# zjwzcx/A-2D-LiDAR-based-SLAM-System-for-Wheeled-Mobile-Robots

Measured on AMD Instinct MI355X. Metric: scans/sec (360-beam ICP + 0.05 m grid update), higher is better.
Workload: dtype f64; 1 GPU; configs[1]: 1000-scan replay (every 5th message of a 10 Hz stream, seed 1), 360 beams, ICP(max_iter=30, tol=0.001) + 400x400@0.05m grid, f64 point buffers; 32 independent replays of the 1000-scan trajectory per step (one slam_replay_dev call: ranges [32, 1000, 360], a map per trajectory); point_buffers=f64, pipeline=0, lanes=2, grid_mode=1, grid_group=16, parallelism=1 trajectory per GPU (32 independent replays of it per step)

## Files before the change

a-2d-lidar-based-slam-system-for-wheeled-mobile-robots_amd/csrc/grid_kernels.hip:

```cpp
#include <hip/hip_runtime.h>

#include <algorithm>
#include <mutex>
#include <utility>
#include <vector>
#include <climits>
#include <cstdio>
#include <cstdlib>
#include <type_traits>

#include "slam_internal.h"
#include "slam_stamps.h"
#include "grid_walk.h"

namespace slam {

__device__ __forceinline__ unsigned cast_ray(uint32_t *__restrict__ pass, uint32_t *__restrict__ hit, int xw, int yw,
                                             int pcx, int pcy, int pox, int poy, bool &first_pending)
{
    Ray r;
    first_pending = false;
    if (!ray_setup(pcx, pcy, pox, poy, r)) return 0u;
    unsigned nvis = 0;
    double error = 0.0;
// ... 448 lines not shown
    int x0 = any ? o[0] : 0, y0 = any ? o[1] : 0, W = any ? o[2] - o[0] + 1 : 0, H = any ? o[3] - o[1] + 1 : 0, cov = 1;
    if (any && !box_fits(o, win_cells)) {
        const int Hd = min(H, 192), Wd = min(W, win_cells / ((Hd + 1) & ~1));
        x0 = min(max(first.pcx - Wd / 2, o[0]), o[2] - Wd + 1);
        y0 = min(max(first.pcy - Hd / 2, o[1]), o[3] - Hd + 1) & ~ymask;
        W = Wd; H = Hd; cov = 0;
    }
    if ((long)W * ((H + 1) >> 1) > win_cells / 2) { atomicOr(g.status, kStatusGuard); W = 0; H = 0; cov = 0; }
    w[0] = x0; w[1] = y0; w[2] = W; w[3] = H; w[4] = cov;
}

__device__ __forceinline__ void flush_window(unsigned *win, uint32_t *pass, int yw, int wx0, int wy0, int W, int Hp2, bool pair64,
                                             bool zero = false)
{
    const int lane = threadIdx.x & 63, wave = threadIdx.x >> 6, nwaves = blockDim.x >> 6;
    const int rot = W > 0 ? (int)((blockIdx.x * 37u + blockIdx.y * 11u) % (unsigned)W) : 0;
    for (int rr = wave; rr < W; rr += nwaves) {
        const int row = rr + rot < W ? rr + rot : rr + rot - W;
        size_t gbase = (size_t)(wx0 + row) * yw + wy0;
        if (pair64 && (wy0 & 1) == 0) {
            for (int d = lane; d < Hp2; d += kWave) {
                unsigned v = win[row * Hp2 + d];
                if (zero) win[row * Hp2 + d] = 0u;
                if (v) atomicAdd(reinterpret_cast<unsigned long long *>(&pass[gbase + 2 * d]),
                                 (unsigned long long)(v & 0xffffu) | ((unsigned long long)(v >> 16) << 32));
            }
            continue;
        }
        for (int d = lane; d < Hp2; d += kWave) {
            unsigned v = win[row * Hp2 + d];
            if (zero) win[row * Hp2 + d] = 0u;
            unsigned p0 = v & 0xffffu, p1 = v >> 16;
            if (p0) atomicAdd(&pass[gbase + 2 * d], p0);
            if (p1) atomicAdd(&pass[gbase + 2 * d + 1], p1);
        }
    }
}

__device__ __forceinline__ void flush_hits(unsigned *win, unsigned short *park, int nrays, uint32_t *hit, int yw, int wx0, int wy0,
                                           int Hs)
{
    __syncthreads();
    for (int k = threadIdx.x; k < nrays; k += blockDim.x) {
        const unsigned c = park[k];
        if (c == kNoHit) continue;
        const unsigned sh = (c & 1u) * 16u;
        const unsigned old = atomicAdd(&win[c >> 1], 1u << sh);
        if ((old >> sh) & 0xffffu) park[k] = (unsigned short)kNoHit;
    }
    __syncthreads();
    for (int k = threadIdx.x; k < nrays; k += blockDim.x) {
        const unsigned c = park[k];
        if (c == kNoHit) continue;
        const unsigned tot = (win[c >> 1] >> ((c & 1u) * 16u)) & 0xffffu;
        const unsigned wx = c / (unsigned)Hs, wy = c - wx * (unsigned)Hs;
        atomicAdd(&hit[(size_t)(wx0 + (int)wx) * yw + (wy0 + (int)wy)], tot);
    }
}

__device__ __forceinline__ void sweep_strip(const unsigned *win, uint32_t *pass, int8_t *pm, int yw, int sx0, int wy0, int SW, int H,
                                            int qrow, unsigned qinv, uint32_t pthr)
{
    const int tid = threadIdx.x, lane = tid & 63, Hp2 = H >> 1, total = SW * qrow;
    constexpr int kBatch = 4;
    for (int q0 = tid; q0 < total; q0 += kBatch * blockDim.x) {
        uint4 p[kBatch];
        uint32_t om[kBatch], d0[kBatch], d1[kBatch];
        size_t at[kBatch];
        bool live[kBatch];
#pragma unroll
        for (int u = 0; u < kBatch; ++u) {
            const int q = q0 + u * (int)blockDim.x;
            d0[u] = d1[u] = 0u;
            if (q < total) {
                const int r = (int)__umulhi((unsigned)q, qinv), c = q - r * qrow;
                const uint2 d = *reinterpret_cast<const uint2 *>(win + (r * Hp2 + 2 * c));
                d0[u] = d.x; d1[u] = d.y;
                at[u] = (size_t)(sx0 + r) * yw + (wy0 + 4 * c);
            }
            const unsigned long long m = __ballot((d0[u] | d1[u]) != 0u);
            live[u] = ((m >> (lane & 60)) & 0xFull) != 0ull;
            if (live[u]) {
                p[u] = *reinterpret_cast<const uint4 *>(pass + at[u]);
                om[u] = *reinterpret_cast<const uint32_t *>(pm + at[u]);
            }
        }
#pragma unroll
        for (int u = 0; u < kBatch; ++u) {
            if (!live[u]) continue;
            const uint32_t d0v = d0[u], d1v = d1[u];
            p[u].x += d0v & 0x7fffu; p[u].y += (d0v >> 16) & 0x7fffu; p[u].z += d1v & 0x7fffu; p[u].w += (d1v >> 16) & 0x7fffu;
            *reinterpret_cast<uint4 *>(pass + at[u]) = p[u];
            if (!(d0v | d1v)) continue;
            const uint32_t o = om[u];
            const uint32_t tb = ((d0v & 0xffffu) ? 1u : 0u) | ((d0v >> 16) ? 0x100u : 0u) | ((d1v & 0xffffu) ? 0x10000u : 0u) | ((d1v >> 16) ? 0x1000000u : 0u);
            const uint32_t fb = ((d0v >> 15) & 1u) | (((d0v >> 31) & 1u) << 8) | (((d1v >> 15) & 1u) << 16) | ((d1v >> 31) << 24);
            const uint32_t was = (o >> 6) & 0x01010101u, fresh = (o >> 4) & 0x01010101u;
            const uint32_t pmax = max(max(p[u].x, p[u].y), max(p[u].z, p[u].w));
            if (((tb & ~was) & (fresh | fb)) != 0u || pmax >= pthr) {
                uint32_t occ = was | fb;
                occ |= (p[u].x >= pthr ? 1u : 0u) | (p[u].y >= pthr ? 0x100u : 0u) | (p[u].z >= pthr ? 0x10000u : 0u) | (p[u].w >= pthr ? 0x1000000u : 0u);
                const uint32_t tm = tb * 255u;
                const uint32_t out = (o & ~tm) | ((occ * 100u) & tm);
                if (out != o) *reinterpret_cast<uint32_t *>(pm + at[u]) = out;
            }
        }
    }
// ... 35 lines not shown
        ctl->phases = 1; ctl->parity = 0;
    }
    const bool sorted = nrays <= sort_cap;
    unsigned short *bins = reinterpret_cast<unsigned short *>(win);
    for (int k = tid; k < 4 * kSortBins; k += blockDim.x) hist[k] = 0;
    __syncthreads();
    STAMP(0);

    win_pass1(g, src, sc, l, s0, cnt, n, sorted, ctl->bbox, ctl->first_bad, [&](int r, int i, bool casts, int quad, int lbin) {
        bins[r] = casts ? (unsigned short)(lbin | (quad << 7) | ((i & 1) << 9)) : (unsigned short)0xffffu;
    });
    if (tid == 0) {
        const int *bb = ctl->bbox;
        if (bb[0] <= bb[2]) {
            int ox0 = INT_MAX, oy0 = INT_MAX, ox1 = INT_MIN, oy1 = INT_MIN;
            for (int k = 0; k < cnt; ++k) { ox0 = min(ox0, sc[k].pcx); ox1 = max(ox1, sc[k].pcx); oy0 = min(oy0, sc[k].pcy); oy1 = max(oy1, sc[k].pcy); }
            quadrant_boxes(bb, ox0, oy0, ox1, oy1, ctl->qbox);
        }
        auto fits = [&](unsigned mask) -> bool { int o[4]; return !box_of(ctl->qbox, mask, g.xw, g.yw, ymask, o) || box_fits(o, win_cells); };
        unsigned part[4] = {0u, 0u, 0u, 0u};
        int nph = 1, parity = 0;
        pick_parts(split != 0, my_half, sorted, fits, part, nph, parity);
        for (int q = 0; q < 4; ++q) ctl->phq[q] = -1;
        for (int ph = 0; ph < nph; ++ph) {
            for (int q = 0; q < 4; ++q)
                if (part[ph] >> q & 1u) ctl->phq[q] = ph;
            int o[4];
            const bool any = box_of(ctl->qbox, part[ph], g.xw, g.yw, ymask, o);
            fit_window(g, any, o, ymask, sc[0], win_cells, ctl->phw[ph]);
        }
        ctl->phases = nph; ctl->parity = parity;
        if (!sorted) { ctl->seg[0] = 0; ctl->seg[1] = nrays; }
    }
    __syncthreads();
    STAMP(1);
    const int phases = ctl->phases;
    if (sorted) {
        const bool parity = ctl->parity != 0;
        for (int r = tid; r < nrays; r += blockDim.x) {
            const unsigned b = bins[r];
            if (b == 0xffffu) continue;
            const int ph = ctl->phq[(b >> 7) & 3u];
            const bool mine = ph >= 0 && (!parity || (int)((b >> 9) & 1u) == my_half);
            const unsigned fin = (unsigned)ph * kSortBins + (b & 127u);
            bins[r] = mine ? (unsigned short)fin : (unsigned short)0xffffu;
            if (mine) atomicAdd(&hist[fin], 1);
        }
        __syncthreads();
        counting_sort<8>(hist, bins, lds.order, nrays, ctl->seg);
    }
    unsigned nvis = 0;
    int W = ctl->phw[0][2], H = ctl->phw[0][3];
    bool covers = ctl->phw[0][4] != 0;
    for (int ph = 0; ph < phases; ++ph) {
        const int seg0 = ctl->seg[ph], seg1 = ctl->seg[ph + 1];
        if (seg0 == seg1) continue;
        const int *o = ctl->phw[ph];
        const int wx0 = o[0], wy0 = o[1];
        W = o[2]; H = o[3]; covers = o[4] != 0;
        const int Hp2 = (H + 1) >> 1;
        __syncthreads();
        if (tid == 0) ctl->next_ray = 0;
        for (int w = tid; w < W * Hp2; w += blockDim.x) win[w] = 0u;
        __syncthreads();
        STAMP(2);
        const unsigned short *ord = sorted ? lds.order + seg0 : nullptr;
        unsigned short *park = sorted && lds_hits ? lds.order + seg0 : nullptr;
        if (covers) nvis += cast_rays<true>(g, src, sc, l, s0, n, seg1 - seg0, &ctl->next_ray, ord, win, wx0, wy0, W, H, Hp2, pass, hit, ctl->first_bad, park);
        else        nvis += cast_rays<false>(g, src, sc, l, s0, n, seg1 - seg0, &ctl->next_ray, ord, win, wx0, wy0, W, H, Hp2, pass, hit, ctl->first_bad, park);
        __syncthreads();
        STAMP(3);
        flush_window(win, pass, g.yw, wx0, wy0, W, Hp2, pair64, park != nullptr);
        if (park) flush_hits(win, park, seg1 - seg0, hit, g.yw, wx0, wy0, 2 * Hp2);
    }
    finish_workgroup(g, &ctl->visits, nvis, tid);
    STAMP(4);
    STAMP_VAL((ctl->parity << 8) | (covers ? 1 : 0) | (phases << 4) | ((unsigned)(W * ((H + 1) & ~1)) << 12));
    STAMP_END(5);
    lds_guard_check(lds.guard, g.status);
}

template <class Src>
__global__ void __launch_bounds__(1024) k_grid_update_own(GridDev g, Src src, int group_size, int sort_cap, int win_cells)
{
    extern __shared__ __attribute__((aligned(16))) char smem[];
    const WinLds lds(smem, group_size, sort_cap, win_cells);
    ScanConst *sc = lds.sc; WinCtl *ctl = lds.ctl; int *hist = lds.hist; unsigned *win = lds.win;
    lds_guard_fill(lds.guard);
    STAMP_DECL;

    const int tid = threadIdx.x, lane = tid & 63, wave = tid >> 6, nwaves = blockDim.x >> 6;
    const int l = blockIdx.y;
    const int s0 = (int)blockIdx.x * group_size;
    const int cnt = min(group_size, src.scans_per_traj() - s0);
    const int gi = src.own_grid(l);
    uint32_t *pass = g.pass + (size_t)gi * g.xw * g.yw, *hit = g.hit + (size_t)gi * g.xw * g.yw;
    int8_t *pm = g.pmap_live + (size_t)gi * g.xw * g.yw;
    const int n = src.n, nrays = cnt * n;

    const bool fused = (g.yw & 3) == 0 && (((size_t)gi * g.xw * g.yw) & 3) == 0;
    const bool pair64 = (g.yw & 1) == 0 && (((size_t)gi * g.xw * g.yw) & 1) == 0;
    const int ymask = fused ? 3 : pair64 ? 1 : 0;
    if (tid < cnt) { src.scan_const(l, s0 + tid, g, sc[tid]); ctl->first_bad[tid] = INT_MAX; }
    if (tid == 0) {
        ctl->bbox[0] = ctl->bbox[1] = INT_MAX; ctl->bbox[2] = ctl->bbox[3] = INT_MIN; ctl->next_ray = 0; ctl->visits = 0ull;
        ctl->strips = 0; ctl->strip_w = 0;
    }
    const bool sorted = nrays <= sort_cap;
    unsigned short *bins = reinterpret_cast<unsigned short *>(win);
    for (int k = tid; k < kSortBins; k += blockDim.x) hist[k] = 0;
    __syncthreads();
    STAMP(0);

    win_pass1(g, src, sc, l, s0, cnt, n, sorted, ctl->bbox, ctl->first_bad, [&](int r, int, bool, int, int lbin) {
        bins[r] = (unsigned short)lbin;
        atomicAdd(&hist[lbin], 1);
    });
    if (tid == 0) {
        int o[4] = {ctl->bbox[0], ctl->bbox[1], ctl->bbox[2], ctl->bbox[3]};
        int *w = ctl->phw[0];
        const bool any = clamp_box(g.xw, g.yw, o, 0);
        if (any && fused && cnt == 1 && nrays < 32768 && g.hit_levels == 1 && (g.yw & 15) == 0) {
            const int ya = o[1] & ~15, Ha = ((o[3] | 15) + 1) - ya, Wb = o[2] - o[0] + 1;
            int S = (int)(((long)Wb * Ha + win_cells - 1) / win_cells), Ws = (Wb + S - 1) / S;
            while ((long)Ws * Ha > win_cells && S < Wb) { ++S; Ws = (Wb + S - 1) / S; }
            if ((long)Ws * Ha <= win_cells) { w[0] = o[0]; w[1] = ya; w[2] = Wb; w[3] = Ha; w[4] = 1; ctl->strips = S; ctl->strip_w = Ws; }
// ... 1594 lines not shown
```

a-2d-lidar-based-slam-system-for-wheeled-mobile-robots_amd/csrc/icp_kernels.hip:

```cpp
#include <hip/hip_fp16.h>
#include <hip/hip_runtime.h>

#include <type_traits>

#include "slam_internal.h"
#include "slam_stamps.h"

namespace slam {

#ifdef SLAM_STAMPS_ICP
__device__ unsigned long long g_polar_lanes[6];
hipError_t debug_polar_lanes(unsigned long long out[6], bool clear)
{
    hipError_t e = hipMemcpyFromSymbol(out, HIP_SYMBOL(g_polar_lanes), sizeof(unsigned long long) * 6);
    if (e == hipSuccess && clear) {
        const unsigned long long zero[6] = {0ull, 0ull, 0ull, 0ull, 0ull, 0ull};
        e = hipMemcpyToSymbol(HIP_SYMBOL(g_polar_lanes), zero, sizeof zero);
    }
    return e;
}
#endif

__device__ __forceinline__ double ld(const double *p, long i) { return p[i]; }
__device__ __forceinline__ double ld(const float *p, long i) { return (double)p[i]; }
// ... 1485 lines not shown
    if (same[0] || same[1]) w[0] = w[1] = w[2] = w[3] = 0.0;
    if (tid == 0) {
        store_transform(T_out + 9 * (long)b, kabsch_from_sums(cax, cay, cbx, cby, w[0], w[1], w[2], w[3]));
    }
}

hipError_t launch_kabsch(const double *src, const double *tar, int B, int n, double *T_out, hipStream_t s)
{
    SLAM_LAUNCH(k_kabsch, dim3(B), dim3(256), 0, s, src, tar, n, T_out);
    return hipGetLastError();
}

template <typename T>
__global__ void __launch_bounds__(256) k_scan_to_points(const float *__restrict__ ranges, const double *__restrict__ cos_t,
                                                        const double *__restrict__ sin_t, long total, int n, int clip_inf,
                                                        T *__restrict__ pts)
{
    for (long e = (long)blockIdx.x * blockDim.x + threadIdx.x; e < total; e += (long)gridDim.x * blockDim.x) {
        long b = e / n;
        int i = (int)(e - b * n);
        double r = (double)ranges[e];
        if (clip_inf && r == INFINITY) r = 30.0;
        st(pts, b * 2 * n + i, cos_t[i] * r);
        st(pts, b * 2 * n + n + i, sin_t[i] * r);
    }
}

hipError_t launch_scan_to_points(const float *ranges, const double *cos_t, const double *sin_t, long total, int n,
                                 int clip_inf, int dtype, void *pts, hipStream_t s)
{
    long blocks = (total + 255) / 256;
    if (blocks > 4096) blocks = 4096;
    if (blocks < 1) blocks = 1;
    switch (dtype) {
    case SLAM_F64:
        SLAM_LAUNCH((k_scan_to_points<double>), dim3(blocks), dim3(256), 0, s, ranges, cos_t, sin_t, total, n, clip_inf, static_cast<double *>(pts));
        break;
    case SLAM_F32:
        SLAM_LAUNCH((k_scan_to_points<float>), dim3(blocks), dim3(256), 0, s, ranges, cos_t, sin_t, total, n, clip_inf, static_cast<float *>(pts));
        break;
    case SLAM_F16:
        SLAM_LAUNCH((k_scan_to_points<__half>), dim3(blocks), dim3(256), 0, s, ranges, cos_t, sin_t, total, n, clip_inf, static_cast<__half *>(pts));
        break;
    default: return hipErrorInvalidValue;
    }
    return hipGetLastError();
}

constexpr int kComposeChunk = 64;
constexpr int kComposeThreads = 256;
constexpr int kComposeBatch = 16;

__global__ void __launch_bounds__(kComposeThreads) k_pose_compose(const double *__restrict__ T, const double *__restrict__ pose0, int n,
                                                                  double *__restrict__ poses)
{
    __shared__ __attribute__((aligned(16))) double dyaw[3][kComposeChunk];
    __shared__ __attribute__((aligned(16))) double thb[2][kComposeChunk];
    __shared__ __attribute__((aligned(16))) double ab[2][kComposeChunk][4];
    __shared__ __attribute__((aligned(16))) double xo[2][2][kComposeChunk];
    __builtin_amdgcn_s_setprio(3);
    const int l = blockIdx.x, tid = threadIdx.x, lane = tid & 63, wave = tid >> 6;
    const double *Tl = T + 9 * (long)l * n;
    double *Pl = poses + 3 * (long)l * n;
    const int nc = (n + kComposeChunk - 1) / kComposeChunk;
    double th = pose0[3 * l + 2];
    double v = pose0[3 * l + (lane & 1)];
    auto load2 = [&](int chunk, int e0, int e1, double &u0, double &u1) {
        const int k = chunk * kComposeChunk + lane;
        const bool in = chunk >= 0 && chunk < nc && k < n;
        u0 = in ? Tl[9 * (long)k + e0] : 0.0;
        u1 = in ? Tl[9 * (long)k + e1] : 0.0;
    };
    double m0 = 0.0, m1 = 0.0;
    if (wave == 2) load2(0, 3, 0, m0, m1);
    if (wave == 3) load2(-2, 2, 5, m0, m1);
    for (int s = 0; s < nc + 4; ++s) {
        if (wave == 0) {
            const int c = s - 1;
            if (c >= 0 && c < nc && lane == 0) {
                const double2 *d2 = reinterpret_cast<const double2 *>(dyaw[c % 3]);
                double2 *o2 = reinterpret_cast<double2 *>(thb[c & 1]);
                double2 cur[kComposeBatch / 2], nxt[kComposeBatch / 2];
#pragma unroll
                for (int u = 0; u < kComposeBatch / 2; ++u) cur[u] = d2[u];
#pragma unroll
                for (int b0 = 0; b0 < kComposeChunk; b0 += kComposeBatch) {
                    if (b0 + kComposeBatch < kComposeChunk) {
#pragma unroll
                        for (int u = 0; u < kComposeBatch / 2; ++u) nxt[u] = d2[(b0 + kComposeBatch) / 2 + u];
                    }
#pragma unroll
                    for (int u = 0; u < kComposeBatch / 2; ++u) {
                        double2 o;
                        o.x = th; th = th + cur[u].x;
                        o.y = th; th = th + cur[u].y;
                        o2[b0 / 2 + u] = o;
                    }
#pragma unroll
                    for (int u = 0; u < kComposeBatch / 2; ++u) cur[u] = nxt[u];
                }
            }
        } else if (wave == 1) {
            const int c = s - 3;
            if (c >= 0 && c < nc && lane < 2) {
                const double2 *p2 = reinterpret_cast<const double2 *>(&ab[c & 1][0][0]) + lane;
                double2 *o2 = reinterpret_cast<double2 *>(xo[c & 1][lane]);
                double2 cur[kComposeBatch], nxt[kComposeBatch];
#pragma unroll
                for (int u = 0; u < kComposeBatch; ++u) cur[u] = p2[2 * u];
#pragma unroll
                for (int b0 = 0; b0 < kComposeChunk; b0 += kComposeBatch) {
                    if (b0 + kComposeBatch < kComposeChunk) {
#pragma unroll
                        for (int u = 0; u < kComposeBatch; ++u) nxt[u] = p2[2 * (b0 + kComposeBatch + u)];
                    }
#pragma unroll
                    for (int u = 0; u < kComposeBatch; u += 2) {
                        double2 o;
                        v = (v + cur[u].x) - cur[u].y;
                        o.x = v;
                        v = (v + cur[u + 1].x) - cur[u + 1].y;
                        o.y = v;
                        o2[(b0 + u) / 2] = o;
                    }
#pragma unroll
                    for (int u = 0; u < kComposeBatch; ++u) cur[u] = nxt[u];
                }
            }
        } else if (wave == 2) {
            double n0, n1;
            load2(s + 1, 3, 0, n0, n1);
            if (s < nc) dyaw[s % 3][lane] = (s * kComposeChunk + lane < n) ? atan2(m0, m1) : 0.0;
            m0 = n0; m1 = n1;
            const int c = s - 4, k = c * kComposeChunk + lane;
            if (c >= 0 && k < n) {
                Pl[3 * (long)k] = xo[c & 1][0][lane];
                Pl[3 * (long)k + 1] = xo[c & 1][1][lane];
            }
        } else {
            double n0, n1;
            load2(s - 1, 2, 5, n0, n1);
            const int c = s - 2, k = c * kComposeChunk + lane;
            if (c >= 0 && c < nc) {
                double a_ = 0.0, b_ = 0.0, c_ = 0.0, d_ = 0.0;
                if (k < n) {
                    const double h = thb[c & 1][lane];
                    const double cs = cos(h), sn = sin(h);
                    a_ = cs * m0; b_ = sn * m1; c_ = sn * m0; d_ = cs * m1;
                    Pl[3 * (long)k + 2] = h + dyaw[c % 3][lane];
                }
                double2 *q = reinterpret_cast<double2 *>(&ab[c & 1][lane][0]);
                q[0] = make_double2(a_, b_);
                q[1] = make_double2(c_, -d_);
            }
            m0 = n0; m1 = n1;
        }
        __syncthreads();
    }
}

__global__ void __launch_bounds__(256) k_pose_step(const double *__restrict__ T, const double *__restrict__ pose0,
                                                   const double *__restrict__ prior, int L, double *__restrict__ poses,
                                                   double *__restrict__ heading_cs)
{
    int l = blockIdx.x * blockDim.x + threadIdx.x;
    if (l >= L) return;
    const double *t = T + 9 * (long)l;
    double m00 = t[0], m10 = t[3], m02 = t[2], m12 = t[5];
    if (prior) {
        const double *p = prior + 6 * (long)l;
        m00 = t[0] * p[0] + t[1] * p[3];
        m10 = t[3] * p[0] + t[4] * p[3];
        m02 = t[0] * p[2] + t[1] * p[5] + t[2];
        m12 = t[3] * p[2] + t[4] * p[5] + t[5];
    }
    double x = pose0[3 * l], y = pose0[3 * l + 1], th = pose0[3 * l + 2];
    double dyaw = atan2(m10, m00);
    double c = cos(th), s = sin(th);
    poses[3 * l] = (x + c * m02) - s * m12;
    poses[3 * l + 1] = (y + s * m02) + c * m12;
    const double th1 = th + dyaw;
    poses[3 * l + 2] = th1;
    if (heading_cs) { heading_cs[2 * l] = cos(th1); heading_cs[2 * l + 1] = sin(th1); }
}

hipError_t launch_pose_compose(const double *T, const double *pose0, int L, int n, double *poses, hipStream_t s,
                               const double *prior, double *heading_cs)
{
    if (prior || heading_cs || (n == 1 && L > 64)) {
        if (n != 1) return hipErrorInvalidValue;
        SLAM_LAUNCH(k_pose_step, dim3((L + 255) / 256), dim3(256), 0, s, T, pose0, prior, L, poses, heading_cs);
        return hipGetLastError();
    }
    SLAM_LAUNCH(k_pose_compose, dim3(L), dim3(kComposeThreads), 0, s, T, pose0, n, poses);
    return hipGetLastError();
}

}
```

a-2d-lidar-based-slam-system-for-wheeled-mobile-robots_amd/csrc/slam_abi.hip:

```cpp
#include <hip/hip_runtime.h>

#include <algorithm>
#include <cmath>
#include <cstdarg>
#include <cstdio>
#include <cstring>
#include <string>
#include <initializer_list>
#include <mutex>
#include <utility>
#include <vector>

#include "slam_internal.h"
#include "slam_stamps.h"

using namespace slam;

namespace {

thread_local std::string g_err;

int fail(int code, const char *fmt, ...)
{
    char buf[512];
// ... 34 lines not shown
}

size_t align_up(size_t v, size_t a = 256) { return (v + a - 1) / a * a; }

struct Arena {
    char *base = nullptr;
    size_t cap = 0, used = 0;
};

struct Pending {
    int kind;
    hipEvent_t e0, e1;
    bool first;
};

}

struct slam_ctx {
    int device = 0;
    hipStream_t stream = nullptr;
    bool own_stream = false;
    Arena staging;
    Arena scratch;
    Arena tiles;
    char *pinned = nullptr;
    size_t pinned_cap = 0;
    int *status = nullptr;
    bool timing = false;
    unsigned timing_mask = ~0u;
    std::vector<hipEvent_t> pool;
    std::vector<Pending> pending;
    double ms[SLAM_K_COUNT] = {0};
    int64_t launches[SLAM_K_COUNT] = {0};
    int grid_mode = 1;
    int grid_group = 0;
    int grid_split = -1;
    int icp_qpt = 0;
    int replay_reset = 0;
    int icp_f32_filter = -1;
    int win_lds_hits = -1;
    int icp_one_wave = -1;
    int raycast_lds = -1;
    int mcl_shape = -1;
    int icp_team = 0;
    int pipeline = 0;
    hipStream_t gstream = nullptr;
    hipStream_t cstream = nullptr;
    hipEvent_t ev_fork = nullptr, ev_join = nullptr, ev_icp = nullptr, ev_pose = nullptr;
    hipEvent_t ev_cast[2] = {nullptr, nullptr};
    const void *cast_poses[2] = {nullptr, nullptr};
    const void *cast_T[2] = {nullptr, nullptr};
    double *pipe_T[2] = {nullptr, nullptr};
    size_t pipe_T_bytes = 0;
    int cast_pos = 0;
    bool gdirty = false;
    bool mgrid = false;
    int particle_chunks = 0;
    hipStream_t pstream = nullptr;
    std::vector<hipEvent_t> pev_pose, pev_cast;
    hipEvent_t pev_join = nullptr;
    bool pdirty = false;
    hipEvent_t ev_order = nullptr;
};

struct slam_grid {
    GridDev d;
    unsigned long long *visits = nullptr;
    size_t state_bytes = 0;
    int8_t *pmap_one = nullptr;
    double *datamap_one = nullptr;
    int8_t *pmap_live = nullptr;
    bool live_dirty = false;
    bool pristine = true;
};

namespace slam {
thread_local LaunchTimer g_launch_timer = {nullptr, nullptr};

hipError_t allow_dynamic_lds(const void *kernel, int bytes)
{
    struct Entry { int dev; const void *kernel; int bytes; };
    static std::mutex mu;
    static std::vector<Entry> done;
    int dev = 0;
    hipError_t e = hipGetDevice(&dev);
    if (e != hipSuccess) return e;
    std::lock_guard<std::mutex> lock(mu);
    Entry *hit = nullptr;
    for (auto &d : done)
        if (d.dev == dev && d.kernel == kernel) hit = &d;
    if (hit && hit->bytes >= bytes) return hipSuccess;
    e = hipFuncSetAttribute(kernel, hipFuncAttributeMaxDynamicSharedMemorySize, bytes);
    if (e != hipSuccess) return e;
    if (hit) hit->bytes = bytes;
    else done.push_back(Entry{dev, kernel, bytes});
    return hipSuccess;
}
}

namespace {

int arena_reserve(slam_ctx *c, Arena &a, size_t bytes)
{
    a.used = 0;
    if (bytes <= a.cap) return SLAM_OK;
    HIPCHK(hipStreamSynchronize(c->stream));
// ... 375 lines not shown
    hipDeviceProp_t prop;
    HIPCHK(hipGetDeviceProperties(&prop, device));
    if (strncmp(prop.gcnArchName, "gfx950", 6) != 0)
        return fail(SLAM_ERR_NODEVICE, "device %d is %s; libslamhip is built for gfx950 (MI355X) only", device,
                    prop.gcnArchName);
    slam_ctx *c = new slam_ctx();
    c->device = device;
    if (stream) {
        c->stream = static_cast<hipStream_t>(stream);
    } else {
        e = hipStreamCreateWithFlags(&c->stream, hipStreamNonBlocking);
        if (e != hipSuccess) {
            delete c;
            return fail(SLAM_ERR_HIP, "hipStreamCreate: %s", hipGetErrorString(e));
        }
        c->own_stream = true;
    }
#ifdef SLAM_STAMPS
    const size_t status_bytes = 256 + (size_t)kStampRecords * 32;
#else
    const size_t status_bytes = 256;
#endif
    e = hipMalloc(reinterpret_cast<void **>(&c->status), status_bytes);
    if (e == hipSuccess) e = hipMemsetAsync(c->status, 0, status_bytes, c->stream);
    if (e == hipSuccess) e = hipStreamSynchronize(c->stream);
    if (e != hipSuccess) {
        delete c;
        return fail(SLAM_ERR_HIP, "context init: %s", hipGetErrorString(e));
    }
    *out = c;
    return SLAM_OK;
}

int slam_destroy(slam_ctx *c)
{
    if (!c) return SLAM_OK;
    (void)hipSetDevice(c->device);
    (void)hipStreamSynchronize(c->stream);
    if (c->pstream) {
        (void)hipStreamSynchronize(c->pstream);
        (void)hipStreamDestroy(c->pstream);
        for (hipEvent_t e : c->pev_pose) (void)hipEventDestroy(e);
        for (hipEvent_t e : c->pev_cast) (void)hipEventDestroy(e);
        if (c->pev_join) (void)hipEventDestroy(c->pev_join);
    }
    if (c->gstream) {
        (void)hipStreamSynchronize(c->cstream);
        (void)hipStreamSynchronize(c->gstream);
        (void)hipStreamDestroy(c->cstream);
        (void)hipStreamDestroy(c->gstream);
        for (hipEvent_t e : {c->ev_fork, c->ev_join, c->ev_icp, c->ev_pose, c->ev_cast[0], c->ev_cast[1]})
            if (e) (void)hipEventDestroy(e);
        for (double *t : c->pipe_T)
            if (t) (void)hipFree(t);
    }
    if (c->ev_order) (void)hipEventDestroy(c->ev_order);
    for (auto &p : c->pending) { (void)hipEventDestroy(p.e0); (void)hipEventDestroy(p.e1); }
    for (auto e : c->pool) (void)hipEventDestroy(e);
    if (c->staging.base) (void)hipFree(c->staging.base);
    if (c->scratch.base) (void)hipFree(c->scratch.base);
    if (c->tiles.base) (void)hipFree(c->tiles.base);
    if (c->pinned) (void)hipHostFree(c->pinned);
    if (c->status) (void)hipFree(c->status);
    if (c->own_stream) (void)hipStreamDestroy(c->stream);
    delete c;
    return SLAM_OK;
}

int slam_synchronize(slam_ctx *c)
{
    TRY(use(c));
    TRY(join_from_grid(c));
    HIPCHK(hipStreamSynchronize(c->stream));
    return SLAM_OK;
}

int slam_stream_order(slam_ctx *c, void *stream, int direction)
{
    TRY(use(c));
    REQUIRE(direction == 0 || direction == 1, "direction is 0 (the stream waits for the context) or 1 (the context waits for the stream)");
    hipStream_t other = static_cast<hipStream_t>(stream);
    if (!c->ev_order) HIPCHK(hipEventCreateWithFlags(&c->ev_order, hipEventDisableTiming));
    if (direction == 0) {
        TRY(join_from_grid(c));
        if (other == c->stream) return SLAM_OK;
        HIPCHK(hipEventRecord(c->ev_order, c->stream));
        HIPCHK(hipStreamWaitEvent(other, c->ev_order, 0));
        return SLAM_OK;
    }
    if (other != c->stream) {
        HIPCHK(hipEventRecord(c->ev_order, other));
        HIPCHK(hipStreamWaitEvent(c->stream, c->ev_order, 0));
    }
    if (c->pipeline) {
        TRY(join_from_grid(c));
        c->mgrid = true;
    }
    return SLAM_OK;
}

int slam_check_status(slam_ctx *c)
{
    TRY(use(c));
    return check_status_sync(c);
}

// ... 460 lines not shown
    g->pristine = true;
    if (g->pmap_live) {
        HIPCHK(hipMemsetAsync(g->pmap_live, 50, (size_t)g->d.G * g->d.xw * g->d.yw, gs(c)));
        g->live_dirty = false;
    }
    if (c->pipeline) c->gdirty = true;
    return SLAM_OK;
}

static int check_grid_update(const char *fn, const slam_grid *g, const double *ox, const double *oy, const double *cx,
                             const double *cy, int B, int n)
{
    REQUIRE_IN(fn, g && ox && oy && cx && cy, "null pointer");
    REQUIRE_IN(fn, B > 0 && n > 0, "sizes must be positive");
    return SLAM_OK;
}

int slam_grid_update_dev(slam_ctx *c, slam_grid *g, const double *ox, const double *oy, const double *cx, const double *cy,
                         int B, int n, const int32_t *grid_of_batch)
{
    TRY(use(c));
    TRY(grid_on_main(c));
    TRY(check_grid_update(__func__, g, ox, oy, cx, cy, B, n));
    g->pristine = false;
    Timed t(c, SLAM_K_GRID);
    CastRequest r;
    r.ox = ox; r.oy = oy; r.cx = cx; r.cy = cy; r.scans = B; r.n = n; r.maps = grid_of_batch;
    r.group = c->grid_group; r.split = c->grid_split; r.lds_hits = c->win_lds_hits;
    const CastPath path = plan_cast(g->d, c->grid_mode, r);
    const size_t need = cast_scratch_bytes(path, r);
    if (need > c->tiles.cap) TRY(arena_reserve(c, c->tiles, need));
    HIPCHK(launch_cast(g->d, path, r, c->tiles.base, c->stream));
    return SLAM_OK;
}

int slam_grid_update(slam_ctx *c, slam_grid *g, const double *ox, const double *oy, const double *cx, const double *cy,
                     int B, int n, const int32_t *grid_of_batch)
{
    TRY(use(c));
    TRY(check_grid_update(__func__, g, ox, oy, cx, cy, B, n));
    if (grid_of_batch)
        for (int b = 0; b < B; ++b) REQUIRE(grid_of_batch[b] >= 0 && grid_of_batch[b] < g->d.G, "grid_of_batch out of range");
    const size_t np = (size_t)B * n;
    double *d_x, *d_y, *d_cx, *d_cy; int32_t *d_g;
    Staging s(c);
    s.in(d_x, ox, np).in(d_y, oy, np).in(d_cx, cx, B).in(d_cy, cy, B).in(d_g, grid_of_batch, B);
    TRY(s.upload());
    TRY(slam_grid_update_dev(c, g, d_x, d_y, d_cx, d_cy, B, n, d_g));
    return check_status_sync(c);
}

static int cast_replay(slam_ctx *c, slam_grid *g, const float *ranges, const double *cos_t, const double *sin_t,
                       const double *poses, const double *centres, int L, int n_scan, int n, const int32_t *got,
                       hipStream_t st)
{
    g->pristine = false;
    CastRequest r;
    r.ranges = ranges; r.cos_t = cos_t; r.sin_t = sin_t; r.poses = poses; r.centres = centres;
    r.L = L; r.scans = n_scan - 1; r.n = n; r.maps = got;
    r.group = c->grid_group; r.split = c->grid_split; r.lds_hits = c->win_lds_hits;
    const CastPath path = plan_cast(g->d, c->grid_mode, r);
    REQUIRE(path != CastPath::Direct || !centres, "grid_mode 0 has no separate ray origins");
    const size_t need = cast_scratch_bytes(path, r);
    if (need > c->tiles.cap) {
        if (c->gstream) HIPCHK(hipStreamSynchronize(c->gstream));
        TRY(arena_reserve(c, c->tiles, need));
    }
    HIPCHK(launch_cast(g->d, path, r, c->tiles.base, st));
    return SLAM_OK;
}

static int check_grid_update_scans(const char *fn, const slam_grid *g, const float *ranges, const double *cos_t,
                                   const double *sin_t, const double *poses, int S, int n)
{
    REQUIRE_IN(fn, g && ranges && cos_t && sin_t && poses, "null pointer");
    REQUIRE_IN(fn, S > 0 && n > 0 && n <= 65535, "bad sizes");
    return SLAM_OK;
}

int slam_grid_update_scans_dev(slam_ctx *c, slam_grid *g, const float *ranges, const double *cos_t, const double *sin_t,
                               const double *poses, const double *centres, int S, int n)
{
    TRY(use(c));
    TRY(grid_on_main(c));
    TRY(check_grid_update_scans(__func__, g, ranges, cos_t, sin_t, poses, S, n));
    Timed t(c, SLAM_K_GRID);
    return cast_replay(c, g, ranges - n, cos_t, sin_t, poses, centres, 1, S + 1, n, nullptr, c->stream);
}

int slam_grid_update_scans(slam_ctx *c, slam_grid *g, const float *ranges, const double *cos_t, const double *sin_t,
                           const double *poses, const double *centres, int S, int n)
{
    TRY(use(c));
    TRY(check_grid_update_scans(__func__, g, ranges, cos_t, sin_t, poses, S, n));
    float *d_r; double *d_c, *d_s, *d_p, *d_o;
    Staging s(c);
    s.in(d_r, ranges, (size_t)S * n).in(d_c, cos_t, n).in(d_s, sin_t, n).in(d_p, poses, (size_t)S * 3).in(d_o, centres, (size_t)S * 2);
    TRY(s.upload());
    TRY(slam_grid_update_scans_dev(c, g, d_r, d_c, d_s, d_p, d_o, S, n));
    return check_status_sync(c);
}

static int refresh_live(slam_ctx *c, slam_grid *g, hipStream_t st)
{
    if (!g->pmap_live || !g->live_dirty) return SLAM_OK;
    Timed t(c, SLAM_K_FINALIZE, st);
    HIPCHK(launch_grid_finalize(g->d, 0, g->d.G, g->pmap_live, st));
    g->live_dirty = false;
    return SLAM_OK;
}

// ... 624 lines not shown
            return fail(SLAM_ERR_INVALID, "line %d does not fit cells_out", b);
    }
    int32_t *d_s, *d_e, *d_l, *d_c; int64_t *d_o;
    Staging s(c);
    s.in(d_s, starts, (size_t)B * 2).in(d_e, ends, (size_t)B * 2).in(d_o, cells_out ? offsets : nullptr, B);
    s.out(d_l, lens_out, B).out(d_c, cells_out, cells_out ? (size_t)total_cells * 2 : 0);
    TRY(s.upload());
    {
        Timed t(c, SLAM_K_BRESENHAM);
        HIPCHK(launch_bresenham(d_s, d_e, B, d_o, d_l, d_c, c->stream));
    }
    return s.download();
}


static int check_replay(const char *fn, const float *ranges, const double *cos_t, const double *sin_t, int L, int n_scan,
                        int n, int dtype, int max_iter, const double *pose0, const double *poses_out)
{
    REQUIRE_IN(fn, ranges && cos_t && sin_t && pose0 && poses_out, "null pointer");
    REQUIRE_IN(fn, L > 0 && n_scan >= 2 && n > 0, "need L > 0, n_scan >= 2, n > 0");
    REQUIRE_IN(fn, max_iter >= 0, "max_iter must be >= 0");
    REQUIRE_IN(fn, dtype_size(dtype), "unknown dtype");
    REQUIRE_IN(fn, n <= 8192, "n too large (max 8192 beams)");
    REQUIRE_IN(fn, (long)L * (n_scan - 1) < (1L << 31), "too many scan pairs for one launch");
    return SLAM_OK;
}

int slam_replay_dev(slam_ctx *c, const float *ranges, const double *cos_t, const double *sin_t, int L, int n_scan, int n,
                    int dtype, int max_iter, double tol, const double *pose0, slam_grid *grid, const int32_t *grid_of_traj,
                    void *pts_ws, double *poses_out, double *T_out, int32_t *iters_out)
{
    TRY(use(c));
    TRY(check_replay(__func__, ranges, cos_t, sin_t, L, n_scan, n, dtype, max_iter, pose0, poses_out));
    (void)pts_ws;
    const long pairs = (long)L * (n_scan - 1);
    const bool piped = c->pipeline && grid;
    double *T = T_out;
    if (!T) {
        if (piped) {
            size_t need = align_up((size_t)pairs * 72);
            if (need > c->pipe_T_bytes) {
                TRY(join_from_grid(c));
                HIPCHK(hipStreamSynchronize(c->stream));
                for (double *&t : c->pipe_T) {
                    if (t) HIPCHK(hipFree(t));
                    t = nullptr;
                    if (hipMalloc(reinterpret_cast<void **>(&t), need) != hipSuccess)
                        return fail(SLAM_ERR_NOMEM, "hipMalloc(%zu bytes) for T", need);
                }
                c->pipe_T_bytes = need;
            }
            T = c->pipe_T[c->cast_pos];
        } else {
            TRY(arena_reserve(c, c->scratch, align_up((size_t)pairs * 72) + 1024));
            T = carve<double>(c->scratch, (size_t)pairs * 9);
        }
    }
    if (c->pipeline)
        for (int k = 0; k < 2; ++k)
            if (c->cast_poses[k] && (c->cast_poses[k] == poses_out || c->cast_T[k] == T)) {
                HIPCHK(hipStreamWaitEvent(c->stream, c->ev_cast[k], 0));
                HIPCHK(hipStreamWaitEvent(c->cstream, c->ev_cast[k], 0));
                c->cast_poses[k] = c->cast_T[k] = nullptr;
            }
    {
        IcpArgs a;
        a.tar = a.src = nullptr; a.prior = nullptr;
        a.ranges = ranges; a.cos_t = cos_t; a.sin_t = sin_t;
        a.tar_scan_stride = a.src_scan_stride = n;
        a.tar_stride = a.src_stride = 0;
        a.ppt = n_scan - 1;
        a.B = (int)pairs; a.n_tar = n; a.n_src = n; a.max_iter = max_iter; a.tol = tol;
        a.T_out = T; a.iters_out = iters_out; a.err_out = nullptr;
        a.status = c->status; a.qpt_pref = c->icp_qpt; a.team_mode = c->icp_team; a.one_wave = c->icp_one_wave; a.f32_filter = c->icp_f32_filter;
        if (grid && c->replay_reset) {
            if (piped || grid->pmap_live) {
                TRY(slam_grid_reset(c, grid));
            } else {
                a.zero_ptr = grid->d.pass; a.zero_bytes = grid->state_bytes;
                grid->pristine = true;
            }
        }
        Timed t(c, SLAM_K_ICP);
        HIPCHK(launch_icp(a, dtype, c->stream));
    }
    if (!piped) {
        {
            Timed t(c, SLAM_K_COMPOSE);
            HIPCHK(launch_pose_compose(T, pose0, L, n_scan - 1, poses_out, c->stream));
        }
        if (grid) {
            TRY(grid_on_main(c));
            Timed t(c, SLAM_K_GRID);
            TRY(cast_replay(c, grid, ranges, cos_t, sin_t, poses_out, nullptr, L, n_scan, n, grid_of_traj, c->stream));
        }
        return SLAM_OK;
    }
    HIPCHK(hipEventRecord(c->ev_icp, c->stream));
    HIPCHK(hipStreamWaitEvent(c->cstream, c->ev_icp, 0));
    {
        Timed t(c, SLAM_K_COMPOSE, c->cstream);
        HIPCHK(launch_pose_compose(T, pose0, L, n_scan - 1, poses_out, c->cstream));
    }
    HIPCHK(hipEventRecord(c->ev_pose, c->cstream));
    HIPCHK(hipStreamWaitEvent(c->gstream, c->ev_pose, 0));
    c->gdirty = true;
    c->mgrid = false;
    {
        Timed t(c, SLAM_K_GRID, c->gstream);
        TRY(cast_replay(c, grid, ranges, cos_t, sin_t, poses_out, nullptr, L, n_scan, n, grid_of_traj, c->gstream));
    }
    HIPCHK(hipEventRecord(c->ev_cast[c->cast_pos], c->gstream));
    c->cast_poses[c->cast_pos] = poses_out;
    c->cast_T[c->cast_pos] = T;
    c->cast_pos ^= 1;
    return SLAM_OK;
}

int slam_replay(slam_ctx *c, const float *ranges, const double *cos_t, const double *sin_t, int L, int n_scan, int n,
                int dtype, int max_iter, double tol, const double *pose0, slam_grid *grid, const int32_t *grid_of_traj,
                double *poses_out, double *T_out, int32_t *iters_out)
{
    TRY(use(c));
    TRY(check_replay(__func__, ranges, cos_t, sin_t, L, n_scan, n, dtype, max_iter, pose0, poses_out));
    if (grid && grid_of_traj)
        for (int l = 0; l < L; ++l) REQUIRE(grid_of_traj[l] >= 0 && grid_of_traj[l] < grid->d.G, "grid_of_traj out of range");
    const size_t pairs = (size_t)L * (n_scan - 1);
    float *d_r; double *d_c, *d_s, *d_0, *d_T, *d_P; int32_t *d_g, *d_it;
    Staging s(c);
    s.in(d_r, ranges, (size_t)L * n_scan * n).in(d_c, cos_t, n).in(d_s, sin_t, n).in(d_0, pose0, (size_t)L * 3)
        .in(d_g, grid ? grid_of_traj : nullptr, L);
    s.out_always(d_T, T_out, pairs * 9).out(d_P, poses_out, pairs * 3).out_always(d_it, iters_out, pairs);
    TRY(s.upload());
    TRY(slam_replay_dev(c, d_r, d_c, d_s, L, n_scan, n, dtype, max_iter, tol, d_0, grid, d_g, nullptr, d_P, d_T, d_it));
    TRY(join_from_grid(c));
    TRY(s.download());
    return check_status_sync(c);
}


static int check_particles(const char *fn, const float *ranges2, const double *cos_t, const double *sin_t, int n, int dtype,
                           const double *pose_prev, int P, int max_iter, const slam_grid *grid, const double *poses_out)
{
    REQUIRE_IN(fn, ranges2 && cos_t && sin_t && pose_prev && poses_out, "null pointer");
    REQUIRE_IN(fn, P > 0 && n > 0 && n <= 8192, "need P > 0 and 0 < n <= 8192");
    REQUIRE_IN(fn, max_iter >= 0, "max_iter must be >= 0");
    REQUIRE_IN(fn, dtype_size(dtype), "unknown dtype");
    REQUIRE_IN(fn, !grid || grid->d.G >= P, "the grid object needs one map per particle");
    return SLAM_OK;
}

int slam_particles_dev(slam_ctx *c, const float *ranges2, const double *cos_t, const double *sin_t, int n, int dtype,
                       const double *prior, const double *pose_prev, int P, int max_iter, double tol, slam_grid *grid,
                       void *pts_ws, double *poses_out, double *T_out, int32_t *iters_out)
{
    TRY(use(c));
    REQUIRE(T_out, "null pointer");
    TRY(check_particles(__func__, ranges2, cos_t, sin_t, n, dtype, pose_prev, P, max_iter, grid, poses_out));
    (void)pts_ws;
    int chunks = c->particle_chunks > 1 ? c->particle_chunks : 1;
    if (!grid || chunks > P) chunks = 1;
    if (chunks == 1) TRY(grid_on_main(c));
    else if (c->pipeline) TRY(join_from_grid(c));
// ... 704 lines not shown
```

Before: 20.01 million scans/s.

## Precompute heading cos/sin in pose compose and skip redundant window zeroing

Pose composition now writes each scan's heading cosine and sine into a buffer that the grid cast reads, so the cast kernel no longer recomputes trig per scan. Separately, the LDS hit window is cleared cell by cell during the hit flush, which lets the next phase's zeroing loop skip the already-clean prefix and use 128-bit stores. This adds a per-pair heading buffer, extra allocation and pipeline synchronization, and relies on the cast path actually consuming heading_cs.

```diff
diff --git a/a-2d-lidar-based-slam-system-for-wheeled-mobile-robots_amd/csrc/grid_kernels.hip b/a-2d-lidar-based-slam-system-for-wheeled-mobile-robots_amd/csrc/grid_kernels.hip
--- a/a-2d-lidar-based-slam-system-for-wheeled-mobile-robots_amd/csrc/grid_kernels.hip
+++ b/a-2d-lidar-based-slam-system-for-wheeled-mobile-robots_amd/csrc/grid_kernels.hip
@@ -524,7 +524,9 @@
     for (int k = threadIdx.x; k < nrays; k += blockDim.x) {
         const unsigned c = park[k];
         if (c == kNoHit) continue;
-        const unsigned tot = (win[c >> 1] >> ((c & 1u) * 16u)) & 0xffffu;
+        unsigned short *cell = reinterpret_cast<unsigned short *>(win) + c;
+        const unsigned tot = *cell;
+        *cell = 0;
         const unsigned wx = c / (unsigned)Hs, wy = c - wx * (unsigned)Hs;
         atomicAdd(&hit[(size_t)(wx0 + (int)wx) * yw + (wy0 + (int)wy)], tot);
     }
@@ -666,6 +668,7 @@
     unsigned nvis = 0;
     int W = ctl->phw[0][2], H = ctl->phw[0][3];
     bool covers = ctl->phw[0][4] != 0;
+    int clean = 0;
     for (int ph = 0; ph < phases; ++ph) {
         const int seg0 = ctl->seg[ph], seg1 = ctl->seg[ph + 1];
         if (seg0 == seg1) continue;
@@ -675,7 +678,10 @@
         const int Hp2 = (H + 1) >> 1;
         __syncthreads();
         if (tid == 0) ctl->next_ray = 0;
-        for (int w = tid; w < W * Hp2; w += blockDim.x) win[w] = 0u;
+        unsigned z = 0u;
+        asm volatile("" : "+v"(z));
+        const uint4 z4 = make_uint4(z, z, z, z);
+        for (int w = (clean & ~3) + 4 * tid; w < W * Hp2; w += 4 * (int)blockDim.x) *reinterpret_cast<uint4 *>(win + w) = z4;
         __syncthreads();
         STAMP(2);
         const unsigned short *ord = sorted ? lds.order + seg0 : nullptr;
@@ -686,6 +692,7 @@
         STAMP(3);
         flush_window(win, pass, g.yw, wx0, wy0, W, Hp2, pair64, park != nullptr);
         if (park) flush_hits(win, park, seg1 - seg0, hit, g.yw, wx0, wy0, 2 * Hp2);
+        clean = park ? max(clean, W * Hp2) : 0;
     }
     finish_workgroup(g, &ctl->visits, nvis, tid);
     STAMP(4);
diff --git a/a-2d-lidar-based-slam-system-for-wheeled-mobile-robots_amd/csrc/icp_kernels.hip b/a-2d-lidar-based-slam-system-for-wheeled-mobile-robots_amd/csrc/icp_kernels.hip
--- a/a-2d-lidar-based-slam-system-for-wheeled-mobile-robots_amd/csrc/icp_kernels.hip
+++ b/a-2d-lidar-based-slam-system-for-wheeled-mobile-robots_amd/csrc/icp_kernels.hip
@@ -1561,7 +1561,7 @@
 constexpr int kComposeBatch = 16;
 
 __global__ void __launch_bounds__(kComposeThreads) k_pose_compose(const double *__restrict__ T, const double *__restrict__ pose0, int n,
-                                                                  double *__restrict__ poses)
+                                                                  double *__restrict__ poses, double *__restrict__ heading_cs)
 {
     __shared__ __attribute__((aligned(16))) double dyaw[3][kComposeChunk];
     __shared__ __attribute__((aligned(16))) double thb[2][kComposeChunk];
@@ -1571,6 +1571,7 @@
     const int l = blockIdx.x, tid = threadIdx.x, lane = tid & 63, wave = tid >> 6;
     const double *Tl = T + 9 * (long)l * n;
     double *Pl = poses + 3 * (long)l * n;
+    double *Hl = heading_cs ? heading_cs + 2 * (long)l * n : nullptr;
     const int nc = (n + kComposeChunk - 1) / kComposeChunk;
     double th = pose0[3 * l + 2];
     double v = pose0[3 * l + (lane & 1)];
@@ -1656,7 +1657,10 @@
                     const double h = thb[c & 1][lane];
                     const double cs = cos(h), sn = sin(h);
                     a_ = cs * m0; b_ = sn * m1; c_ = sn * m0; d_ = cs * m1;
-                    Pl[3 * (long)k + 2] = h + dyaw[c % 3][lane];
+                    const double hn = h + dyaw[c % 3][lane];
+                    Pl[3 * (long)k + 2] = hn;
+                    if (heading_cs && k > 0) *reinterpret_cast<double2 *>(Hl + 2 * (long)(k - 1)) = make_double2(cs, sn);
+                    if (heading_cs && k == n - 1) *reinterpret_cast<double2 *>(Hl + 2 * (long)k) = make_double2(cos(hn), sin(hn));
                 }
                 double2 *q = reinterpret_cast<double2 *>(&ab[c & 1][lane][0]);
                 q[0] = make_double2(a_, b_);
@@ -1696,12 +1700,12 @@
 hipError_t launch_pose_compose(const double *T, const double *pose0, int L, int n, double *poses, hipStream_t s,
                                const double *prior, double *heading_cs)
 {
-    if (prior || heading_cs || (n == 1 && L > 64)) {
+    if (prior || (heading_cs && n == 1) || (n == 1 && L > 64)) {
         if (n != 1) return hipErrorInvalidValue;
         SLAM_LAUNCH(k_pose_step, dim3((L + 255) / 256), dim3(256), 0, s, T, pose0, prior, L, poses, heading_cs);
         return hipGetLastError();
     }
-    SLAM_LAUNCH(k_pose_compose, dim3(L), dim3(kComposeThreads), 0, s, T, pose0, n, poses);
+    SLAM_LAUNCH(k_pose_compose, dim3(L), dim3(kComposeThreads), 0, s, T, pose0, n, poses, heading_cs);
     return hipGetLastError();
 }
 
diff --git a/a-2d-lidar-based-slam-system-for-wheeled-mobile-robots_amd/csrc/slam_abi.hip b/a-2d-lidar-based-slam-system-for-wheeled-mobile-robots_amd/csrc/slam_abi.hip
--- a/a-2d-lidar-based-slam-system-for-wheeled-mobile-robots_amd/csrc/slam_abi.hip
+++ b/a-2d-lidar-based-slam-system-for-wheeled-mobile-robots_amd/csrc/slam_abi.hip
@@ -110,6 +110,8 @@
     const void *cast_T[2] = {nullptr, nullptr};
     double *pipe_T[2] = {nullptr, nullptr};
     size_t pipe_T_bytes = 0;
+    double *pipe_cs[2] = {nullptr, nullptr};
+    size_t pipe_cs_bytes = 0;
     int cast_pos = 0;
     bool gdirty = false;
     bool mgrid = false;
@@ -591,6 +593,8 @@
         for (hipEvent_t e : {c->ev_fork, c->ev_join, c->ev_icp, c->ev_pose, c->ev_cast[0], c->ev_cast[1]})
             if (e) (void)hipEventDestroy(e);
         for (double *t : c->pipe_T)
+            if (t) (void)hipFree(t);
+        for (double *t : c->pipe_cs)
             if (t) (void)hipFree(t);
     }
     if (c->ev_order) (void)hipEventDestroy(c->ev_order);
@@ -1157,11 +1161,11 @@
 
 static int cast_replay(slam_ctx *c, slam_grid *g, const float *ranges, const double *cos_t, const double *sin_t,
                        const double *poses, const double *centres, int L, int n_scan, int n, const int32_t *got,
-                       hipStream_t st)
+                       hipStream_t st, const double *heading_cs = nullptr)
 {
     g->pristine = false;
     CastRequest r;
-    r.ranges = ranges; r.cos_t = cos_t; r.sin_t = sin_t; r.poses = poses; r.centres = centres;
+    r.ranges = ranges; r.cos_t = cos_t; r.sin_t = sin_t; r.poses = poses; r.centres = centres; r.heading_cs = heading_cs;
     r.L = L; r.scans = n_scan - 1; r.n = n; r.maps = got;
     r.group = c->grid_group; r.split = c->grid_split; r.lds_hits = c->win_lds_hits;
     const CastPath path = plan_cast(g->d, c->grid_mode, r);
@@ -1892,13 +1896,32 @@
             }
             T = c->pipe_T[c->cast_pos];
         } else {
-            TRY(arena_reserve(c, c->scratch, align_up((size_t)pairs * 72) + 1024));
+            TRY(arena_reserve(c, c->scratch, align_up((size_t)pairs * 72) + (grid ? align_up((size_t)pairs * 16) : 0) + 1024));
             T = carve<double>(c->scratch, (size_t)pairs * 9);
         }
-    }
+    } else if (grid && !piped)
+        TRY(arena_reserve(c, c->scratch, align_up((size_t)pairs * 16) + 1024));
+    double *heading_cs = nullptr;
+    if (piped) {
+        const size_t need = align_up((size_t)pairs * 16);
+        if (need > c->pipe_cs_bytes) {
+            TRY(join_from_grid(c));
+            HIPCHK(hipStreamSynchronize(c->stream));
+            for (double *&t : c->pipe_cs) {
+                if (t) HIPCHK(hipFree(t));
+                t = nullptr;
+                c->pipe_cs_bytes = 0;
+                if (hipMalloc(reinterpret_cast<void **>(&t), need) != hipSuccess)
+                    return fail(SLAM_ERR_NOMEM, "hipMalloc(%zu bytes) for the headings", need);
+            }
+            c->pipe_cs_bytes = need;
+        }
+        heading_cs = c->pipe_cs[c->cast_pos];
+    } else if (grid)
+        heading_cs = carve<double>(c->scratch, (size_t)pairs * 2);
     if (c->pipeline)
         for (int k = 0; k < 2; ++k)
-            if (c->cast_poses[k] && (c->cast_poses[k] == poses_out || c->cast_T[k] == T)) {
+            if (c->cast_poses[k] && (c->cast_poses[k] == poses_out || c->cast_T[k] == T || (piped && k == c->cast_pos))) {
                 HIPCHK(hipStreamWaitEvent(c->stream, c->ev_cast[k], 0));
                 HIPCHK(hipStreamWaitEvent(c->cstream, c->ev_cast[k], 0));
                 c->cast_poses[k] = c->cast_T[k] = nullptr;
@@ -1927,12 +1950,12 @@
     if (!piped) {
         {
             Timed t(c, SLAM_K_COMPOSE);
-            HIPCHK(launch_pose_compose(T, pose0, L, n_scan - 1, poses_out, c->stream));
+            HIPCHK(launch_pose_compose(T, pose0, L, n_scan - 1, poses_out, c->stream, nullptr, heading_cs));
         }
         if (grid) {
             TRY(grid_on_main(c));
             Timed t(c, SLAM_K_GRID);
-            TRY(cast_replay(c, grid, ranges, cos_t, sin_t, poses_out, nullptr, L, n_scan, n, grid_of_traj, c->stream));
+            TRY(cast_replay(c, grid, ranges, cos_t, sin_t, poses_out, nullptr, L, n_scan, n, grid_of_traj, c->stream, heading_cs));
         }
         return SLAM_OK;
     }
@@ -1940,7 +1963,7 @@
     HIPCHK(hipStreamWaitEvent(c->cstream, c->ev_icp, 0));
     {
         Timed t(c, SLAM_K_COMPOSE, c->cstream);
-        HIPCHK(launch_pose_compose(T, pose0, L, n_scan - 1, poses_out, c->cstream));
+        HIPCHK(launch_pose_compose(T, pose0, L, n_scan - 1, poses_out, c->cstream, nullptr, heading_cs));
     }
     HIPCHK(hipEventRecord(c->ev_pose, c->cstream));
     HIPCHK(hipStreamWaitEvent(c->gstream, c->ev_pose, 0));
@@ -1948,7 +1971,7 @@
     c->mgrid = false;
     {
         Timed t(c, SLAM_K_GRID, c->gstream);
-        TRY(cast_replay(c, grid, ranges, cos_t, sin_t, poses_out, nullptr, L, n_scan, n, grid_of_traj, c->gstream));
+        TRY(cast_replay(c, grid, ranges, cos_t, sin_t, poses_out, nullptr, L, n_scan, n, grid_of_traj, c->gstream, heading_cs));
     }
     HIPCHK(hipEventRecord(c->ev_cast[c->cast_pos], c->gstream));
     c->cast_poses[c->cast_pos] = poses_out;
```

After: 19.98 million scans/s. Within noise of the previous version (-0.2%).
